# ArisKonidaris/OMLDM

Hardware: AMD Instinct MI355X
Metric: training examples/sec (whole node) + p50 predict latency, linear SVM 1/2/4/8 GPU (higher is better)
Workload: dtype fp32

## Files before the change

csrc/kernels/linear_scan3.hip:

```cpp
#include "common.h"
#include "hash_dev.h"
#include "seq_common.h"

#include <mutex>
#include <unordered_map>

namespace omldm {

typedef float f32x4 __attribute__((ext_vector_type(4)));

namespace s3 {
constexpr int CH = 64;
#ifndef OMLDM_S3_NH
#define OMLDM_S3_NH 11
#endif
constexpr int NH = OMLDM_S3_NH;
constexpr int NT = 64 * (NH + 1);
constexpr int WPE = (NH + 1 + 3) / 4;
constexpr int NHA = NH;
constexpr int GS = CH + 4;
constexpr int MAXF = 32;
constexpr int NF = (MAXF + NHA - 1) / NHA;
constexpr int KNMAX = 32;
constexpr int NJ = (KNMAX + NHA - 1) / NHA;
constexpr int MAT = CH * CH;
constexpr int RMAX = 8192;
constexpr int WS = 8;
constexpr int DS = KNMAX;
constexpr uint32_t F_TG = 1u;
constexpr uint32_t F_INIT = 2u;
constexpr uint32_t F_SCAT = 4u;
constexpr uint32_t F_SIGN = 8u;
constexpr uint32_t F_PRES = 16u;
constexpr uint32_t F_TAB = F_TG | F_INIT | F_SCAT;
constexpr int LID_SHIFT = 10;
}

template <int KN>
__host__ __device__ constexpr int s3_prep_floats() {
  return 2 * s3::MAT + s3::CH + KN * s3::CH + 3 * s3::CH;
}
template <int KN>
__host__ __device__ constexpr int s3_prep_y() {
  return 2 * s3::MAT + s3::CH + KN * s3::CH;
}
template <int KN>
__host__ __device__ constexpr int s3_prep_sg() {
  return s3_prep_y<KN>() + s3::CH;
}
template <int KN>
__host__ __device__ constexpr int s3_prep_hh() {
  return s3_prep_y<KN>() + 2 * s3::CH;
}
__device__ __forceinline__ float s3_shrink(int shr, float r, float tbase, int i, float y) {
  if (shr == 0 || y != y) return 1.f;
  if (shr == 2) {
    const float T = tbase + (float)i;
    return (T - 1.f) / T;
  }
  return r;
}

__device__ __forceinline__ void spoke_rows(int s, int R, int B, int& t0, int& t1) {
  const long long a = (long long)s * R;
  t0 = a > B ? B : (int)a;
  t1 = (a + R) > B ? B : (int)(a + R);
}

__global__ __launch_bounds__(256) void s3_slots_kernel(const void* __restrict__ src, int B,
                                                       int dc, int dn, uint32_t span, int hashed,
                                                       int cbase, int* __restrict__ slotsT) {
  __shared__ int tile[256][s3::MAXF + 1];
  const int r0 = blockIdx.x * 256, tid = threadIdx.x;
  const int nr = min(256, B - r0);
  for (int i = tid; i < nr * dc; i += 256) {
    const int r = i / dc, f = i - r * dc;
    int slot;
    if (hashed == 2) {
      const uint32_t v = reinterpret_cast<const uint16_t*>(src)[(size_t)r0 * dc + i];
      slot = v == 0xFFFFu ? -1
                          : (int)(((uint32_t)cbase + (uint32_t)f * span + (v & 0x7FFFu)) |
                                  ((v & 0x8000u) << 16));
    } else {
      const uint32_t v = reinterpret_cast<const uint32_t*>(src)[(size_t)r0 * dc + i];
      slot = hashed ? (int)v : hash_token_dev(v, f, dn, span);
    }
    tile[r][f] = slot;
  }
  __syncthreads();
  if (tid < nr)
    for (int f = 0; f < dc; ++f) slotsT[(size_t)f * B + r0 + tid] = tile[tid][f];
}

namespace s3 {
constexpr int FT = 1024;
constexpr int HCAP = 12288;
constexpr int RPT = RMAX / FT;
}

__global__ __launch_bounds__(s3::FT) void s3_flags_kernel(const int* __restrict__ slotsT, int B,
                                                          int R, uint32_t* __restrict__ meta,
                                                          int* __restrict__ lidcount, int enc,
                                                          int* __restrict__ l2s, long long gs) {
  __shared__ int hkey[s3::HCAP];
  __shared__ uint32_t hfirst[s3::HCAP];
  __shared__ uint32_t hlast[s3::HCAP];
  __shared__ int s_cnt, s_base;
  const int f = blockIdx.x, s = blockIdx.y, tid = threadIdx.x, lane = tid & 63;
  int t0, t1;
  spoke_rows(s, R, B, t0, t1);
  const int n = t1 - t0;
  if (n <= 0) return;
  for (int i = tid; i < s3::HCAP; i += s3::FT) {
    hkey[i] = -1;
    hfirst[i] = 0xFFFFFFFFu;
    hlast[i] = 0u;
  }
  if (tid == 0) s_cnt = 0;
  __syncthreads();
  const int* col = slotsT + (size_t)f * B + t0;
// ... 57 lines not shown
      const int ch = i >> 6;
      m = v[q] < 0 ? s3::F_SIGN : 0u;
      if ((last >> 6) - (first >> 6) >= 2) {
        if (ch > (first >> 6)) m |= s3::F_TG;
        if (i == first) m |= s3::F_INIT;
        if ((last >> 6) >= ch + 2) m |= s3::F_SCAT;
        m |= (uint32_t)(base + hkey[h[q]]) << s3::LID_SHIFT;
        if (l2s && lloc[q] >= 0) l2s[(size_t)s * gs + base + lloc[q]] = v[q] & 0x7fffffff;
      } else if (enc) {
        m |= s3::F_PRES | ((uint32_t)(v[q] & 0x7fffffff) << s3::LID_SHIFT);
      }
    }
    meta[(size_t)f * B + t0 + i] = m;
  }
}

__device__ __forceinline__ void s3_gram_colscale(float (*scol)[s3::CH], float cscale,
                                                 const void* __restrict__ yv, int y8, int t0,
                                                 int t1, int c, int tid) {
  if (cscale == 0.f || tid >= 2 * s3::CH) return;
  const int d = tid / s3::CH, r = tid - d * s3::CH;
  const int row = t0 + (c - d) * s3::CH + r;
  const float y = (c - d >= 0 && row < t1) ? load_y(yv, row, y8) : 0.f;
  scol[d][r] = y == y ? cscale * y : 0.f;
}

template <int KN>
__global__ __launch_bounds__(256) void s3_gram_kernel(const int* __restrict__ slotsT, int dc,
                                                      const float* __restrict__ num, int dn,
                                                      const void* __restrict__ yv, int y8,
                                                      int B, int R, int bias, int affine,
                                                      float kadd, float* __restrict__ prep,
                                                      int nchs, int shr, float shr_r,
                                                      float cscale) {
  const int c = blockIdx.x, s = blockIdx.y;
  int t0, t1;
  spoke_rows(s, R, B, t0, t1);
  if (t0 + c * s3::CH >= t1) return;
  constexpr int PF = s3_prep_floats<KN>();
  float* out = prep + ((size_t)s * nchs + c) * PF;
  __shared__ alignas(16) int sl[2][s3::MAXF][s3::CH + 4];
  __shared__ float xn[2][s3::CH][KN + 1];
  __shared__ float sa[s3::CH];
  __shared__ float scol[2][s3::CH];
  const int tid = threadIdx.x;
  s3_gram_colscale(scol, cscale, yv, y8, t0, t1, c, tid);
  for (int i = tid; i < 2 * dc * s3::CH; i += 256) {
    const int d = i / (dc * s3::CH), rem = i - d * dc * s3::CH;
    const int f = rem / s3::CH, r = rem - f * s3::CH;
    const int cc = c - d, row = t0 + cc * s3::CH + r;
    sl[d][f][r] = (cc >= 0 && row < t1) ? slotsT[(size_t)f * B + row] : -1;
  }
  for (int i = tid; i < 2 * s3::CH * KN; i += 256) {
    const int d = i / (s3::CH * KN), rem = i - d * s3::CH * KN;
    const int r = rem / KN, j = rem - r * KN;
    const int cc = c - d, row = t0 + cc * s3::CH + r;
    float x = 0.f;
    if (cc >= 0 && row < t1) x = j < dn ? num[(size_t)row * dn + j] : ((bias && j == dn) ? 1.f : 0.f);
    xn[d][r][j] = x;
  }
  __syncthreads();
  if (tid < s3::CH) {
    float n2 = 0.f;
    for (int j = 0; j < KN; ++j) n2 = fmaf(xn[0][tid][j], xn[0][tid][j], n2);
    for (int f = 0; f < dc; ++f) n2 += sl[0][f][tid] != -1 ? 1.f : 0.f;
    const bool live = t0 + c * s3::CH + tid < t1;
    const float yt = live ? load_y(yv, t0 + c * s3::CH + tid, y8) : __builtin_nanf("");
    float a = 0.f, g = 1.f;
    if (live) {
      a = affine == 1 ? (n2 > 0.f ? -1.f / (n2 + kadd) : 0.f)
        : affine == 2 ? (yt == yt ? yt : 0.f)
        : affine == 3 ? (n2 > 0.f ? 1.f / (2.f * n2 + kadd) : 0.f) : 1.f;
      if (affine == 1 && shr == 1 && yt == yt) g = 1.f / shr_r;
    }
    sa[tid] = affine == 3 ? (live ? 1.f : 0.f) : a * g;
    out[2 * s3::MAT + tid] = a;
    out[s3_prep_y<KN>() + tid] = yt;
  }
  for (int i = tid; i < KN * s3::CH; i += 256) {
    const int j = i / s3::CH, r = i - j * s3::CH;
    out[2 * s3::MAT + s3::CH + i] = xn[0][r][j];
  }
  __syncthreads();
  const int bi = tid >> 4, bj = tid & 15;
#pragma unroll 1
  for (int d = 0; d < 2; ++d) {
    float acc[4][4] = {};
    if (c - d >= 0 && !(d == 0 && bj > bi)) {
      int cnt[4][4] = {};
      for (int f = 0; f < dc; ++f) {
        const int4 a4 = *reinterpret_cast<const int4*>(&sl[0][f][4 * bi]);
        const int4 b4 = *reinterpret_cast<const int4*>(&sl[d][f][4 * bj]);
        const int av[4] = {a4.x, a4.y, a4.z, a4.w}, bv[4] = {b4.x, b4.y, b4.z, b4.w};
#pragma unroll
        for (int i = 0; i < 4; ++i) {
          const int a = av[i] == -1 ? 0x7ffffffe : av[i];
#pragma unroll
          for (int j = 0; j < 4; ++j) {
            const int x = a ^ bv[j];
            cnt[i][j] += (x & 0x7fffffff) ? 0 : (x < 0 ? -1 : 1);
          }
        }
      }
#pragma unroll
      for (int i = 0; i < 4; ++i)
#pragma unroll
        for (int j = 0; j < 4; ++j) acc[i][j] = (float)cnt[i][j];
      for (int q = 0; q < KN; ++q) {
        float xa[4], xb[4];
#pragma unroll
        for (int i = 0; i < 4; ++i) {
          xa[i] = xn[0][4 * bi + i][q];
          xb[i] = xn[d][4 * bj + i][q];
        }
#pragma unroll
        for (int i = 0; i < 4; ++i)
#pragma unroll
          for (int j = 0; j < 4; ++j) acc[i][j] = fmaf(xa[i], xb[j], acc[i][j]);
      }
    }
#pragma unroll
    for (int i = 0; i < 4; ++i) {
      const int t = 4 * bi + i;
      const float a = sa[t];
      float4 v = make_float4(a * acc[i][0], a * acc[i][1], a * acc[i][2], a * acc[i][3]);
      if (cscale != 0.f) {
        v.x *= scol[d][4 * bj + 0];
        v.y *= scol[d][4 * bj + 1];
        v.z *= scol[d][4 * bj + 2];
        v.w *= scol[d][4 * bj + 3];
      }
      if (d == 0) {
        if (4 * bj + 0 >= t) v.x = 0.f;
        if (4 * bj + 1 >= t) v.y = 0.f;
        if (4 * bj + 2 >= t) v.z = 0.f;
        if (4 * bj + 3 >= t) v.w = 0.f;
      }
      *reinterpret_cast<float4*>(&out[d * s3::MAT + t * s3::CH + 4 * bj]) = v;
    }
  }
}

__device__ int g_s3_gram_ablate = 0;

template <int KN>
__global__ __launch_bounds__(256) void s3_gram_mfma_kernel(const int* __restrict__ slotsT, int dc,
                                                           const float* __restrict__ num, int dn,
                                                           const void* __restrict__ yv, int y8,
                                                           int B, int R, int bias, int affine,
                                                           float kadd, float* __restrict__ prep,
                                                           int nchs, int shr, float shr_r,
                                                           float cscale) {
  typedef float f32x16 __attribute__((ext_vector_type(16)));
  const int c = blockIdx.x, s = blockIdx.y;
  int t0, t1;
  spoke_rows(s, R, B, t0, t1);
  if (t0 + c * s3::CH >= t1) return;
  constexpr int PF = s3_prep_floats<KN>();
  float* out = prep + ((size_t)s * nchs + c) * PF;
  __shared__ alignas(16) int sl[2][s3::MAXF][s3::CH + 4];
  __shared__ float xn[2][s3::CH][KN + 1];
  __shared__ float sa[s3::CH];
  __shared__ float scol[2][s3::CH];
  const int tid = threadIdx.x, lane = tid & 63, wave = tid >> 6;
  s3_gram_colscale(scol, cscale, yv, y8, t0, t1, c, tid);
  constexpr int NSL = 2 * s3::MAXF * s3::CH / 256, NXN = 2 * s3::CH * KN / 256;
  int sv[NSL];
  float xv[NXN];
#pragma unroll
  for (int u = 0; u < NSL; ++u) {
    const int i = tid + 256 * u;
    const int d = i / (s3::MAXF * s3::CH), rem = i - d * s3::MAXF * s3::CH;
    const int f = rem / s3::CH, r = rem - f * s3::CH;
    const int cc = c - d, row = t0 + cc * s3::CH + r;
    const bool ok = f < dc && cc >= 0 && row < t1;
    const int v = slotsT[ok ? (size_t)f * B + row : 0];
    sv[u] = ok ? v : -1;
  }
#pragma unroll
  for (int u = 0; u < NXN; ++u) {
    const int i = tid + 256 * u;
    const int d = i / (s3::CH * KN), rem = i - d * s3::CH * KN;
    const int r = rem / KN, j = rem - r * KN;
    const int cc = c - d, row = t0 + cc * s3::CH + r;
    const bool in = cc >= 0 && row < t1;
    const float x = dn > 0 ? num[(in && j < dn) ? (size_t)row * dn + j : 0] : 0.f;
    xv[u] = in ? (j < dn ? x : ((bias && j == dn) ? 1.f : 0.f)) : 0.f;
  }
#pragma unroll
  for (int u = 0; u < NSL; ++u) {
    const int i = tid + 256 * u;
    const int d = i / (s3::MAXF * s3::CH), rem = i - d * s3::MAXF * s3::CH;
    sl[d][rem / s3::CH][rem % s3::CH] = sv[u];
  }
#pragma unroll
  for (int u = 0; u < NXN; ++u) {
    const int i = tid + 256 * u;
    const int d = i / (s3::CH * KN), rem = i - d * s3::CH * KN;
    xn[d][rem / KN][rem % KN] = xv[u];
  }
  __syncthreads();
  if (tid < s3::CH) {
    float n2 = 0.f;
    for (int j = 0; j < KN; ++j) n2 = fmaf(xn[0][tid][j], xn[0][tid][j], n2);
    for (int f = 0; f < dc; ++f) n2 += sl[0][f][tid] != -1 ? 1.f : 0.f;
    const bool live = t0 + c * s3::CH + tid < t1;
    const float yt = live ? load_y(yv, t0 + c * s3::CH + tid, y8) : __builtin_nanf("");
    float a = 0.f, g = 1.f;
    if (live) {
      a = affine == 1 ? (n2 > 0.f ? -1.f / (n2 + kadd) : 0.f)
        : affine == 2 ? (yt == yt ? yt : 0.f)
        : affine == 3 ? (n2 > 0.f ? 1.f / (2.f * n2 + kadd) : 0.f) : 1.f;
      if (affine == 1 && shr == 1 && yt == yt) g = 1.f / shr_r;
    }
    sa[tid] = affine == 3 ? (live ? 1.f : 0.f) : a * g;
    out[2 * s3::MAT + tid] = a;
    out[s3_prep_y<KN>() + tid] = yt;
  }
  for (int i = tid; i < KN * s3::CH; i += 256) {
    const int j = i / s3::CH, r = i - j * s3::CH;
    out[2 * s3::MAT + s3::CH + i] = xn[0][r][j];
  }
  __syncthreads();
  const int l31 = lane & 31, hi = lane >> 5;
#pragma unroll 1
  for (int pass = 0; pass < 2; ++pass) {
    const int d = pass == 0 ? 1 : 0;
    const int I0 = pass == 0 ? 32 * (wave >> 1) : ((wave == 1 || wave == 2) ? 32 : 0);
    const int J0 = pass == 0 ? 32 * (wave & 1) : (wave >= 2 ? 32 : 0);
    const bool zero = (pass == 1 && wave == 3) || c - d < 0;
    f32x16 acc;
#pragma unroll
    for (int g = 0; g < 16; ++g) acc[g] = 0.f;
    const int abl = g_s3_gram_ablate;
    if (!zero) {
      int cnt[16];
#pragma unroll
      for (int g = 0; g < 16; ++g) cnt[g] = 0;
      for (int f = 0; f < ((abl & 1) ? 0 : dc); ++f) {
        const int b = sl[d][f][J0 + l31];
#pragma unroll
        for (int g = 0; g < 4; ++g) {
          const int4 a4 = *reinterpret_cast<const int4*>(&sl[0][f][I0 + 8 * g + 4 * hi]);
          const int av[4] = {a4.x, a4.y, a4.z, a4.w};
#pragma unroll
          for (int e = 0; e < 4; ++e) {
            const int a = av[e] == -1 ? 0x7ffffffe : av[e];
            const int x = a ^ b;
            cnt[4 * g + e] += (x & 0x7fffffff) ? 0 : (x < 0 ? -1 : 1);
          }
        }
      }
#pragma unroll
      for (int g = 0; g < 16; ++g) acc[g] = (float)cnt[g];
      if (!(abl & 2)) {
#pragma unroll
        for (int k0 = 0; k0 < KN; k0 += 2)
          acc = __builtin_amdgcn_mfma_f32_32x32x2f32(xn[0][I0 + l31][k0 + hi],
                                                     xn[d][J0 + l31][k0 + hi], acc, 0, 0, 0);
      }
    }
    if (abl & 4) continue;
#pragma unroll
    for (int g = 0; g < 16; ++g) {
      const int t = I0 + (g & 3) + 8 * (g >> 2) + 4 * hi, col = J0 + l31;
      float v = sa[t] * acc[g];
      if (cscale != 0.f) v *= scol[d][col];
      if (d == 0 && col >= t) v = 0.f;
      out[d * s3::MAT + t * s3::CH + col] = v;
    }
  }
}

template <int KN>
__global__ __launch_bounds__(64) void s3_sigma_kernel(float* __restrict__ prep, int nchs, int B,
                                                      int R, int shr, float shr_r, float tbase,
                                                      float* __restrict__ sig) {
  constexpr int PF = s3_prep_floats<KN>();
  const int s = blockIdx.x, lane = threadIdx.x;
  int t0, t1;
  spoke_rows(s, R, B, t0, t1);
  const int n = t1 - t0;
  if (n <= 0) return;
  float* P0 = prep + (size_t)s * nchs * PF;
  auto at = [&](int i) -> float* { return P0 + (size_t)(i >> 6) * PF + (i & 63); };
  const int L = (n + 63) / 64, i0 = lane * L, i1 = min(n, i0 + L);
  float pr = 1.f;
  for (int i = i0; i < i1; ++i) pr *= s3_shrink(shr, shr_r, tbase, i, at(i)[s3_prep_y<KN>()]);
  float incl = pr;
#pragma unroll
  for (int d = 1; d < 64; d <<= 1) {
    const float o = __shfl_up(incl, d, 64);
    if (lane >= d) incl *= o;
  }
  float sg = __shfl_up(incl, 1, 64);
  if (lane == 0) sg = 1.f;
  for (int i = i0; i < i1; ++i) {
    float* b = at(i);
    b[s3_prep_sg<KN>()] = sg;
    sg *= s3_shrink(shr, shr_r, tbase, i, b[s3_prep_y<KN>()]);
    b[s3_prep_hh<KN>()] = 1.f / sg;
  }
  const int tail = (64 - (n & 63)) & 63;
  if (lane < tail) {
    float* b = at(n + lane);
    b[s3_prep_sg<KN>()] = 1.f;
    b[s3_prep_hh<KN>()] = 1.f;
  }
  if (lane == 63) sig[s] = incl;
}

struct S3Smem {
  alignas(16) float G[2][s3::CH][s3::GS];
  alignas(16) float X1[2][s3::CH][s3::GS];
  float part[2][s3::NHA][s3::CH];
  float cb[2][s3::CH];
  int last;
};

template <int RULE>
struct S3Cand {
  float lo, hi, d;
  __device__ __forceinline__ float operator()(float u, const SeqParams& p, float y) const {
    if constexpr (RULE == kSeqHinge) {
      return __builtin_amdgcn_fmed3f(u, lo, hi);
    } else if constexpr (RULE == kSeqEps) {
      return __builtin_amdgcn_fmed3f(u, 0.f, hi) + __builtin_amdgcn_fmed3f(u + d, lo, 0.f);
    } else if constexpr (RULE == kSeqPegasos) {
      return u < lo ? hi : 0.f;
    } else {
      return hi * __builtin_amdgcn_rcpf(1.f + __expf(lo * u));
    }
  }
};

__device__ unsigned long long* g_s3_stamps;
__device__ int g_s3_debug;
__device__ unsigned long long* g_s3mc_dbg;
__device__ int g_s3_comb_err;
__device__ int g_s3_dense_order = 0;
__device__ int g_s3_hprio = 0;

typedef __attribute__((address_space(1))) unsigned long long s3_gu64;
template <bool B>
struct S3Tag {
  static constexpr bool value = B;
};
struct S3Comb {
  const int* lidcount;
  unsigned long long* gran;
  uint32_t epoch;
  int S_act;
// ... 286 lines not shown
        const int sl = i < n ? slot[u] : 0;
        d[u] -= i < n ? (cb.wbf ? s3_w16(w, sl) : w[sl]) : 0.f;
      }
    }
#pragma unroll
    for (int u = 0; u < FB; ++u) {
      const int i = i0 + u * s3::NT;
      if (i < n && d[u] != 0.f) atomicAdd(&cb.dacc[slot[u]], sc * d[u]);
    }
  }
}

__device__ __forceinline__ void s3_spoke_end(bool tail, const int* __restrict__ slotsT, int dc,
                                             int B, int R, const S3Comb& cb,
                                             const float* __restrict__ ws,
                                             const float* __restrict__ wsd, int dn, int dim,
                                             const SeqParams& p, S3Smem& sm, int s) {
  if (tail) {
    __syncthreads();
    s3_combine_spoke(slotsT, dc, B, R, cb, sm, s, 0, 1);
  }
  s3_scan_arrive(cb, ws, wsd, dn, dim, p, sm);
}

template <int RULE, int KN, bool RARE>
__device__ __forceinline__ void s3_scan_body(
    int bid, int nblk, int tail, S3Smem& sm, float* tab,
    const int* __restrict__ slotsT, const uint32_t* __restrict__ meta, int dc, int dn,
    const void* __restrict__ yv, int B, int R, const float* __restrict__ prep, int nchs,
    const float* __restrict__ w, int dim, float* __restrict__ aglob, int cap, long long gstride,
    const S3Comb& cb, float* __restrict__ ws, float* __restrict__ wsd, const SeqParams& p,
    unsigned long long* __restrict__ rgran) {
  constexpr int PF = s3_prep_floats<KN>();
  if (bid >= cb.S_act) {
    if (RARE && bid < 2 * cb.S_act) {
      s3_rare(slotsT, dc, B, R, w, cb, rgran, sm, bid - cb.S_act);
      if (cb.inscan == 2) s3_fold_pres(meta, dc, B, R, cb, bid - cb.S_act);
      if (tail == 2) {
        __syncthreads();
        s3_combine_spoke(slotsT, dc, B, R, cb, sm, bid - cb.S_act, 0, 1);
      }
      return;
    }
    s3_combine(slotsT, dc, B, R, cb, sm, (RARE ? 2 : 1) * cb.S_act, bid, nblk, cb.cns);
    return;
  }
  const int tid = threadIdx.x;
  const int wave = __builtin_amdgcn_readfirstlane(tid >> 6), lane = tid & 63;
  const int s = bid;
  int t0, t1;
  spoke_rows(s, R, B, t0, t1);
  if (t0 >= t1) {
    if (tid < s3::WS) ws[(size_t)s * s3::WS + tid] = 0.f;
    if (tid < s3::DS) wsd[(size_t)s * s3::DS + tid] = 0.f;
    s3_scan_arrive(cb, ws, wsd, dn, dim, p, sm);
    return;
  }
  const int nch = (t1 - t0 + s3::CH - 1) / s3::CH;
  const float* P0 = prep + (size_t)s * nchs * PF;
  auto chunk_prep = [&](int k) { return P0 + (size_t)k * PF; };
  float* ag = aglob + (size_t)s * gstride;

  unsigned long long* stamps = g_s3_stamps;
  const bool dbg_gather = g_s3_debug == 1;
  unsigned long long st_acc[12] = {};
  unsigned long long st_t = stamps ? clock64() : 0;
  auto stamp = [&](int k) {
    if (stamps) {
      const unsigned long long now = clock64();
      st_acc[k] += now - st_t;
      st_t = now;
    }
  };

  if (wave == 0) {
    __builtin_amdgcn_s_setprio(3);
    float loss = 0.f, nex = 0.f, mist = 0.f, sqe = 0.f;
    float f1 = 0.f;
    float ynx = chunk_prep(0)[s3_prep_y<KN>() + lane];
    float anx = chunk_prep(0)[2 * s3::MAT + lane];
    const bool shr = p.shr != 0;
    float snx = shr ? chunk_prep(0)[s3_prep_sg<KN>() + lane] : 1.f;
    float hnx = shr ? chunk_prep(0)[s3_prep_hh<KN>() + lane] : 1.f;
    for (int k = -1; k <= nch; ++k) {
      if (k >= 0 && k < nch) {
        const int b = k & 1;
        const int row = t0 + k * s3::CH + lane;
        const bool valid = row < t1 && ynx == ynx;
        const float y = valid ? ynx : 0.f;
        const float a = valid ? anx : 0.f;
        const float sg = valid ? snx : 1.f, hh = valid ? hnx : 1.f;
        if (k + 1 < nch) {
          ynx = chunk_prep(k + 1)[s3_prep_y<KN>() + lane];
          anx = chunk_prep(k + 1)[2 * s3::MAT + lane];
          if (shr) {
            snx = chunk_prep(k + 1)[s3_prep_sg<KN>() + lane];
            hnx = chunk_prep(k + 1)[s3_prep_hh<KN>() + lane];
          }
        }
        float m0 = 0.f;
#pragma unroll
        for (int q = 0; q < s3::NHA; ++q) m0 += sm.part[b][q][lane];
        S3Cand<RULE> cf;
        float u, bc = 0.f;
        const float inv = -a;
        if constexpr (RULE == kSeqHinge) {
          bc = y * inv * hh;
          cf.lo = y < 0.f ? -p.cclip * hh : 0.f;
          cf.hi = y < 0.f ? 0.f : (y > 0.f ? p.cclip * hh : 0.f);
          u = fmaf(a * (sg * hh), m0, bc) + f1;
        } else if constexpr (RULE == kSeqEps) {
          bc = (y - p.eps) * inv * hh;
          cf.d = 2.f * p.eps * inv * hh;
          cf.lo = valid ? -p.cclip * hh : 0.f;
          cf.hi = valid ? p.cclip * hh : 0.f;
          u = fmaf(a * (sg * hh), m0, bc) + f1;
        } else if constexpr (RULE == kSeqPegasos) {
          const float T = p.tbase + (float)(row - t0);
          cf.lo = valid ? 1.f / sg : 0.f;
          cf.hi = valid ? y * hh / (p.lam * T) : 0.f;
          u = fmaf(a, m0, 0.f) + f1;
        } else {
          cf.lo = y * sg;
          cf.hi = p.lr * y * hh;
          u = m0 + f1;
        }
        const float* grow = &sm.G[b][lane][0];
        const float* xrow = &sm.X1[b ^ 1][lane][0];
        float gg[s3::CH], xx[s3::CH];
#pragma unroll
        for (int t4 = 0; t4 < s3::CH; t4 += 4) {
          const float4 g4 = *reinterpret_cast<const float4*>(grow + t4);
          const float4 x4 = *reinterpret_cast<const float4*>(xrow + t4);
          gg[t4] = g4.x, gg[t4 + 1] = g4.y, gg[t4 + 2] = g4.z, gg[t4 + 3] = g4.w;
          xx[t4] = x4.x, xx[t4 + 1] = x4.y, xx[t4 + 2] = x4.z, xx[t4 + 3] = x4.w;
        }
        stamp(8);
        float n1 = 0.f;
        auto chain = [&](auto step) {
#pragma unroll
          for (int t = 0; t < s3::CH; ++t) {
            const float ct = readlane_f(step(u), t);
            u = fmaf(ct, gg[t], u);
            n1 = fmaf(ct, xx[t], n1);
            asm volatile("" : "+v"(u), "+v"(n1));
          }
        };
        if constexpr (RULE == kSeqLogistic) {
          if (!shr) {
            const float lo2 = y * 1.44269504088896341f;
            chain([&](float v) {
              return __builtin_amdgcn_rcpf(1.f + __builtin_amdgcn_exp2f(lo2 * v));
            });
          } else {
            chain([&](float v) { return cf(v, p, y); });
          }
        } else {
          chain([&](float v) { return cf(v, p, y); });
        }
        stamp(9);
        const float c = cf(u, p, y);
        sm.cb[b][lane] = c;
        if (row < t1 && cb.inscan != 1)
          __hip_atomic_store((s3_gu64*)(cb.gran + row),
                             ((unsigned long long)cb.epoch << 32) | __float_as_uint(c),
                             __ATOMIC_RELAXED, __HIP_MEMORY_SCOPE_AGENT);
        if (valid) {
          float m;
          if constexpr (RULE == kSeqLogistic) m = sg * u;
          else if constexpr (RULE == kSeqPegasos) m = sg * y * u;
          else m = inv > 0.f ? (bc - u) * __builtin_amdgcn_rcpf(inv * hh) : 0.f;
          seq_stats<RULE>(m, y, p, loss, mist, sqe);
          nex += 1.f;
        }
        f1 = n1;
      }
      stamp(0);
      __syncthreads();
      stamp(1);
    }
    if (stamps && lane == 0)
      for (int q = 0; q < 12; ++q)
        if (q < 2 || q >= 8) atomicAdd(&stamps[(size_t)s * 16 + q], st_acc[q]);
    loss = wave_sum(loss);
    nex = wave_sum(nex);
    mist = wave_sum(mist);
    sqe = wave_sum(sqe);
    if (lane == 0) {
      float* wr = ws + (size_t)s * s3::WS;
      wr[0] = loss;
      wr[1] = nex;
      wr[2] = mist;
      wr[3] = sqe;
      wr[4] = 1.f;
      wr[5] = 0.f;
      wr[6] = 0.f;
      wr[7] = 0.f;
    }
    if (cb.inscan) s3_inscan_flush<RARE>(cb, tab, ag, cap, w, s);
    s3_spoke_end(tail == 1, slotsT, dc, B, R, cb, ws, wsd, dn, dim, p, sm, s);
    return;
  }

  const int q = wave - 1, r = lane;
  const int swave = g_s3_debug >= 16 ? g_s3_debug - 16 : 1;
  if (g_s3_hprio) {
    if (q >= 7) __builtin_amdgcn_s_setprio(2);
    else if (q >= 3) __builtin_amdgcn_s_setprio(1);
  }
  const int qd = g_s3_dense_order ? s3::NHA - 1 - q : q;
  const int kd = dn + (p.bias ? 1 : 0);
  const int hl = q * 64 + lane;
  const bool inscan = cb.inscan != 0, inscan1 = cb.inscan == 1;
  const uint32_t tmask = inscan ? s3::F_TAB : s3::F_SCAT;
  const float isc = inscan1 ? cb.inv_p * (cb.sig ? cb.sig[s] : 1.f) : 0.f;
  float wn[s3::NJ], w0[s3::NJ];
#pragma unroll
  for (int i = 0; i < s3::NJ; ++i) {
    const int j = qd + s3::NHA * i;
    const int jw = j < dn ? j : dim - 1;
    const float wj = cb.wbf ? s3_w16(w, jw) : w[jw];
    w0[i] = (j < KN && (j < dn || (p.bias && j == dn))) ? wj : 0.f;
    wn[i] = w0[i];
  }
  constexpr int NV4 = (2 * s3::MAT / 4 + 64 * s3::NHA - 1) / (64 * s3::NHA);
  struct Set {
    int cs[s3::NF];
    uint32_t cm[s3::NF];
    float g[s3::NF];
    f32x4 v[NV4];
    float xs[s3::NJ], xc[s3::NJ];
    unsigned long long rg;
  };
  uint32_t p1[s3::NF], p2[s3::NF];
  const unsigned long long want = (unsigned long long)cb.epoch;
  bool dead = false;
  auto load_rare = [&](int ch) -> unsigned long long {
    const int row = t0 + ch * s3::CH + r;
    const bool ok = RARE && q == 0 && ch >= 0 && ch < nch && row < t1;
    return ok ? __hip_atomic_load((s3_gu64*)(rgran + row), __ATOMIC_RELAXED,
                                  __HIP_MEMORY_SCOPE_AGENT)
              : (want << 32);
  };
  auto load_words = [&](int ch, Set& S) {
    if constexpr (RARE) {
      S.rg = load_rare(ch);
#pragma unroll
      for (int i = 0; i < s3::NF; ++i) {
        const int f = q + s3::NHA * i;
        const int row = t0 + ch * s3::CH + r;
        const bool ok = ch >= 0 && ch < nch && f < dc && row < t1;
        const uint32_t mm = meta[ok ? (size_t)f * B + row : 0];
        S.cm[i] = ok ? mm : 0u;
        S.cs[i] = ok && (mm & (s3::F_TG | s3::F_INIT)) ? 0 : -1;
      }
      return;
    }
#pragma unroll
    for (int i = 0; i < s3::NF; ++i) {
      const int f = q + s3::NHA * i;
      const int row = t0 + ch * s3::CH + r;
      const bool ok = ch >= 0 && ch < nch && f < dc && row < t1;
      const size_t at = ok ? (size_t)f * B + row : 0;
      const int sl = slotsT[at];
      const uint32_t mm = meta[at];
      S.cs[i] = ok ? sl : -1;
      S.cm[i] = ok ? mm : 0u;
    }
  };
  auto issue_gathers = [&](Set& S) {
    if constexpr (RARE) return;
    if (cb.wbf) {
#pragma unroll
      for (int i = 0; i < s3::NF; ++i) {
        const bool glob = !RARE && S.cs[i] != -1 && !(S.cm[i] & s3::F_TG);
        S.g[i] = s3_w16(w, (glob && !dbg_gather) ? (S.cs[i] & 0x7fffffff) : 0);
      }
      return;
    }
#pragma unroll
    for (int i = 0; i < s3::NF; ++i) {
      const bool glob = !RARE && S.cs[i] != -1 && !(S.cm[i] & s3::F_TG);
      S.g[i] = w[(glob && !dbg_gather) ? (S.cs[i] & 0x7fffffff) : 0];
    }
  };
  auto issue_staging = [&](int ch, Set& S) {
#pragma unroll
    for (int u = 0; u < NV4; ++u) {
      const int i = min(hl + 64 * s3::NHA * u, 2 * s3::MAT / 4 - 1);
      const int mtx = i >> 10, e = i & 1023;
      const int kc = max(0, min(ch + mtx, nch - 1));
      S.v[u] = reinterpret_cast<const f32x4*>(chunk_prep(kc) + mtx * s3::MAT)[e];
    }
  };
  constexpr int NJK = (KN + s3::NHA - 1) / s3::NHA;
  auto load_dense = [&](int ch, float* xd) {
#pragma unroll
    for (int i = 0; i < NJK; ++i) {
      const int j = qd + s3::NHA * i;
      const bool ok = j < KN && ch >= 0 && ch < nch;
      const int jc = j < KN ? j : 0, cc = max(0, min(ch, nch - 1));
      const float v = chunk_prep(cc)[2 * s3::MAT + s3::CH + jc * s3::CH + r];
      xd[i] = ok ? v : 0.f;
    }
  };
  auto body = [&](auto spill_tag, int k, Set& CUR, Set& NXT) {
    constexpr bool SPILL = decltype(spill_tag)::value;
    const int cn = k + 1, ks = k - 1;
    if (wave == swave) stamp(7);
    load_words(cn + 1, NXT);
    issue_staging(cn + 1, NXT);
    load_dense(ks + 1, NXT.xs);
    load_dense(cn + 1, NXT.xc);
    if (wave == swave) stamp(3);
    if (ks >= 0) {
      const float cv = sm.cb[ks & 1][r];
#pragma unroll
      for (int i = 0; i < s3::NF; ++i) {
        const uint32_t m = p2[i];
        const bool sc = (m & tmask) != 0u && cv != 0.f;
        const bool dr = inscan1 && (m & s3::F_PRES) != 0u && cv != 0.f;
        if (__builtin_amdgcn_ballot_w64(sc || dr) == 0ull) continue;
        const int lid = (int)(m >> s3::LID_SHIFT);
        const float val = (m & s3::F_SIGN) ? -cv : cv;
        if (dr) atomicAdd(&cb.dacc[lid], val * isc);
        if (sc) {
          if constexpr (SPILL) {
            if (lid < cap) atomicAdd(&tab[lid], val);
            else atomicAdd(&ag[lid - cap], val);
          } else {
            atomicAdd(&tab[lid], val);
          }
        }
      }
#pragma unroll
      for (int i = 0; i < NJK; ++i) {
        const int j = qd + s3::NHA * i;
        if (j < kd) wn[i] += wave_sum(cv * CUR.xs[i]);
      }
    }
    if (wave == swave) stamp(6);
    if (cn < nch) {
      float base = 0.f;
#pragma unroll
      for (int i = 0; i < NJK; ++i) base = fmaf(CUR.xc[i], wn[i], base);
      if constexpr (RARE) {
        if (q == 0) {
          for (unsigned spins = 0;
               __builtin_amdgcn_ballot_w64((CUR.rg >> 32) != want) != 0ull;) {
            if (dead || ++spins > s3::SPIN_MAX) {
              if (!dead && r == 0) atomicExch(&g_s3_comb_err, 2);
              dead = true;
              break;
            }
            __builtin_amdgcn_s_sleep(1);
            CUR.rg = load_rare(cn);
          }
          base += (CUR.rg >> 32) == want ? __uint_as_float((uint32_t)CUR.rg) : 0.f;
        }
      }
      if constexpr (!SPILL) {
        float tv[s3::NF];
#pragma unroll
        for (int i = 0; i < s3::NF; ++i) {
          const uint32_t m = CUR.cm[i];
          const bool tg = CUR.cs[i] != -1 && (m & s3::F_TG);
          tv[i] = 0.f;
          if (tg) tv[i] = tab[(int)(m >> s3::LID_SHIFT)];
        }
#pragma unroll
        for (int i = 0; i < s3::NF; ++i) {
          const uint32_t m = CUR.cm[i];
          const bool here = CUR.cs[i] != -1;
          const bool tg = here && (m & s3::F_TG), init = here && !tg && (m & s3::F_INIT);
          const float val = tg ? tv[i] : (RARE ? 0.f : CUR.g[i]);
          if (init) tab[(int)(m >> s3::LID_SHIFT)] = val;
          if (here && (!RARE || tg)) base += (m & s3::F_SIGN) ? -val : val;
        }
      }
#pragma unroll
      for (int i = 0; SPILL && i < s3::NF; ++i) {
        const uint32_t m = CUR.cm[i];
        const bool here = CUR.cs[i] != -1;
        const int lid = (int)(m >> s3::LID_SHIFT);
        const bool tg = here && (m & s3::F_TG), init = here && !tg && (m & s3::F_INIT);
        float val = RARE ? 0.f : CUR.g[i];
        if (!SPILL || __builtin_amdgcn_ballot_w64((tg || init) && lid >= cap) == 0ull) {
          if (tg) val = tab[lid];
          if (init) tab[lid] = val;
        } else if constexpr (SPILL) {
          if (tg) val = lid < cap ? tab[lid] : __hip_atomic_load(&ag[lid - cap], __ATOMIC_RELAXED,
                                                                 __HIP_MEMORY_SCOPE_WORKGROUP);
          if (init) {
            if (lid < cap) tab[lid] = val;
            else __hip_atomic_store(&ag[lid - cap], val, __ATOMIC_RELAXED,
                                    __HIP_MEMORY_SCOPE_WORKGROUP);
          }
          asm volatile("s_waitcnt vmcnt(0)" ::: "memory");
        }
        if (here && (!RARE || tg)) base += (m & s3::F_SIGN) ? -val : val;
      }
      sm.part[cn & 1][q][r] = base;
    }
    if (wave == swave) stamp(4);
#pragma unroll
    for (int u = 0; u < NV4; ++u) {
      const int i = hl + 64 * s3::NHA * u;
      const int mtx = i >> 10, e = i & 1023;
      if (i < 2 * s3::MAT / 4 && cn + mtx < nch) {
        const int row = e >> 4, col = (e & 15) * 4;
        float* dst = mtx == 0 ? &sm.G[cn & 1][row][col] : &sm.X1[(cn + 1) & 1][row][col];
        *reinterpret_cast<f32x4*>(dst) = CUR.v[u];
      }
    }
    issue_gathers(NXT);
#pragma unroll
    for (int i = 0; i < s3::NF; ++i) {
      p2[i] = p1[i];
      p1[i] = CUR.cm[i];
    }
    if (wave == swave) stamp(5);
    __syncthreads();
  };

  Set A, Bs;
#pragma unroll
  for (int i = 0; i < s3::NF; ++i) p1[i] = p2[i] = 0u;
  load_words(0, A);
  issue_staging(0, A);
  load_dense(-2, A.xs);
  load_dense(0, A.xc);
  issue_gathers(A);
  if (cb.lidcount[s] <= cap) {
    for (int k = -1; k <= nch; k += 2) {
      body(S3Tag<false>{}, k, A, Bs);
      if (k + 1 <= nch) body(S3Tag<false>{}, k + 1, Bs, A);
    }
  } else {
    for (int k = -1; k <= nch; k += 2) {
      body(S3Tag<true>{}, k, A, Bs);
      if (k + 1 <= nch) body(S3Tag<true>{}, k + 1, Bs, A);
    }
  }
  if (stamps && lane == 0 && wave == swave)
    for (int k = 2; k < 8; ++k) atomicAdd(&stamps[(size_t)s * 16 + k], st_acc[k]);
#pragma unroll
  for (int i = 0; i < s3::NJ; ++i) {
    const int j = qd + s3::NHA * i;
    if (lane == 0 && j < KN) wsd[(size_t)s * s3::DS + j] = wn[i] - w0[i];
  }
  if (q == 0 && lane >= KN && lane < s3::DS) wsd[(size_t)s * s3::DS + lane] = 0.f;
  if (cb.inscan) s3_inscan_flush<RARE>(cb, tab, ag, cap, w, s);
  s3_spoke_end(tail == 1, slotsT, dc, B, R, cb, ws, wsd, dn, dim, p, sm, s);
}

constexpr int kS3MaxPipes = 16;
struct S3Pipe {
  const float* w;
  float* aglob;
  float* ws;
  float* wsd;
  unsigned long long* rgran;
  S3Comb cb;
  SeqParams p;
};
struct S3Pipes {
  int M;
  int ncomb;
  int tail;
  const unsigned long long* wflag;
  unsigned long long wepoch;
  S3Pipe pipe[kS3MaxPipes];
};

__global__ void s3_signal_kernel(unsigned long long* flag, unsigned long long epoch) {
  if (threadIdx.x == 0)
    __hip_atomic_store(flag, epoch, __ATOMIC_RELEASE, __HIP_MEMORY_SCOPE_AGENT);
}

__device__ __forceinline__ void s3_wait_prep(const unsigned long long* flag,
                                             unsigned long long epoch) {
  if (flag == nullptr) return;
  if (threadIdx.x == 0) {
    for (unsigned spins = 0;
         __hip_atomic_load(flag, __ATOMIC_RELAXED, __HIP_MEMORY_SCOPE_AGENT) < epoch;) {
      if (++spins > s3::SPIN_MAX) {
        atomicExch(&g_s3_comb_err, 3);
        break;
      }
      __builtin_amdgcn_s_sleep(2);
    }
    __builtin_amdgcn_fence(__ATOMIC_ACQUIRE, "agent");
  }
  __syncthreads();
}

template <int RULE, int KN, bool RARE>
__global__ __launch_bounds__(s3::NT, s3::WPE) __attribute__((amdgpu_waves_per_eu(s3::WPE, s3::WPE))) void s3_scan_kernel(
    const int* __restrict__ slotsT, const uint32_t* __restrict__ meta, int dc, int dn,
    const void* __restrict__ yv, int B, int R, const float* __restrict__ prep, int nchs,
    int dim, int cap, long long gstride, int S_act, S3Pipes pp) {
  __shared__ S3Smem sm;
  extern __shared__ float tab[];
  const int nblk = s3_nper(S_act, RARE, pp.ncomb, pp.pipe[0].cb.cns);
  const int pi = (int)blockIdx.x / nblk, local = (int)blockIdx.x % nblk;
  s3_wait_prep(pp.wflag, pp.wepoch);
  int bid;
  if (RARE && local < S_act) bid = S_act + local;
  else if (RARE && local < 2 * S_act) bid = local - S_act;
  else bid = local;
  const S3Pipe& P = pp.pipe[pi];
  s3_scan_body<RULE, KN, RARE>(bid, nblk, pp.tail, sm, tab, slotsT, meta,
// ... 330 lines not shown
  auto w0_at = [&](int i, int c) {
    const int j = q + s3::NHA * i;
    const int key = j < dn ? j : dim - 1;
    const bool real = j < KN && (j < dn || (bias && j == dn));
    return real ? A.Wt[(size_t)key * A.kp + c] : 0.f;
  };
#pragma unroll
  for (int i = 0; i < NJK0; ++i)
#pragma unroll
    for (int c = 0; c < K; ++c) wn[c][i] = w0_at(i, c);
  constexpr int NV4 = (2 * s3::MAT / 4 + 64 * s3::NHA - 1) / (64 * s3::NHA);
  constexpr int NJK = (KN + s3::NHA - 1) / s3::NHA;
  struct Set {
    int cs[s3::NF];
    uint32_t cm[s3::NF];
    float g[s3::NF][K];
    f32x4 v[NV4];
    float xs[s3::NJ], xc[s3::NJ];
  };
  uint32_t p1[s3::NF], p2[s3::NF];
  auto load_words = [&](int ch, Set& S) {
#pragma unroll
    for (int i = 0; i < s3::NF; ++i) {
      const int f = q + s3::NHA * i;
      const int row = t0 + ch * s3::CH + r;
      const bool ok = ch >= 0 && ch < nch && f < dc && row < t1;
      const size_t at = ok ? (size_t)f * B + row : 0;
      const int sl = slotsT[at];
      const uint32_t mm = meta[at];
      S.cs[i] = ok ? sl : -1;
      S.cm[i] = ok ? mm : 0u;
    }
  };
  auto issue_gathers = [&](Set& S) {
#pragma unroll
    for (int i = 0; i < s3::NF; ++i) {
      const bool glob = S.cs[i] != -1 && !(S.cm[i] & s3::F_TG);
      const float* src = A.Wt + (size_t)(glob ? (S.cs[i] & 0x7fffffff) : 0) * A.kp;
      if constexpr (K >= 4) {
#pragma unroll
        for (int c4 = 0; c4 < K; c4 += 4) {
          const float4 v = *reinterpret_cast<const float4*>(src + c4);
          S.g[i][c4] = v.x, S.g[i][c4 + 1] = v.y, S.g[i][c4 + 2] = v.z, S.g[i][c4 + 3] = v.w;
        }
      } else {
        const float2 v = *reinterpret_cast<const float2*>(src);
        S.g[i][0] = v.x, S.g[i][1] = v.y;
      }
    }
  };
  auto issue_staging = [&](int ch, Set& S) {
#pragma unroll
    for (int u = 0; u < NV4; ++u) {
      const int i = min(hl + 64 * s3::NHA * u, 2 * s3::MAT / 4 - 1);
      const int mtx = i >> 10, e = i & 1023;
      const int kc = max(0, min(ch + mtx, nch - 1));
      S.v[u] = reinterpret_cast<const f32x4*>(chunk_prep(kc) + mtx * s3::MAT)[e];
    }
  };
  auto load_dense = [&](int ch, float* xd) {
#pragma unroll
    for (int i = 0; i < NJK; ++i) {
      const int j = q + s3::NHA * i;
      const bool ok = j < KN && ch >= 0 && ch < nch;
      const int jc = j < KN ? j : 0, cc = max(0, min(ch, nch - 1));
      const float v = chunk_prep(cc)[2 * s3::MAT + s3::CH + jc * s3::CH + r];
      xd[i] = ok ? v : 0.f;
    }
  };
  auto tab_add = [&](auto spill_tag, int lid, int c, float v) {
    constexpr bool SPILL = decltype(spill_tag)::value;
    if (!SPILL || lid < capid) atomicAdd(&tab[lid * K + c], v);
    else atomicAdd(&ag[(size_t)(lid - capid) * K + c], v);
  };
  unsigned long long* const hdbg = g_s3mc_dbg;
  unsigned long long h_sc = 0, h_mg = 0, h_st = 0, h_wt = 0;
  constexpr bool LEAN = K >= 8;
  auto store_staging = [&](int cn, const Set& S) {
#pragma unroll
    for (int u = 0; u < NV4; ++u) {
      const int i = hl + 64 * s3::NHA * u;
      const int mtx = i >> 10, e = i & 1023;
      if (i < 2 * s3::MAT / 4 && cn + mtx < nch) {
        const int row = e >> 4, col = (e & 15) * 4;
        float* dst = mtx == 0 ? &sm.G[cn & 1][row][col] : &sm.X1[(cn + 1) & 1][row][col];
        *reinterpret_cast<f32x4*>(dst) = S.v[u];
      }
    }
  };
  auto body = [&](auto spill_tag, int k, Set& CUR, Set& NXT) {
    constexpr bool SPILL = decltype(spill_tag)::value;
    const int cn = k + 1, ks = k - 1;
    const unsigned long long ha = hdbg ? __builtin_amdgcn_s_memtime() : 0;
    load_words(cn + 1, NXT);
    if constexpr (LEAN) {
      issue_staging(cn, CUR);
      if constexpr (K < 16) issue_gathers(CUR);
    } else {
      issue_staging(cn + 1, NXT);
    }
    load_dense(ks + 1, NXT.xs);
    load_dense(cn + 1, NXT.xc);
    if (ks >= 0) {
      const float tv = sm.tau[ks & 1][r];
      const int rc = sm.rr[ks & 1][r];
      const float yf = chunk_prep(ks)[s3_prep_y<KN>() + r];
      const int yc = (yf == yf && yf >= 0.f && yf < (float)A.nclass) ? (int)yf : -1;
#pragma unroll
      for (int i = 0; i < s3::NF; ++i) {
        const uint32_t m = p2[i];
        const bool sc = (m & s3::F_SCAT) != 0u && tv != 0.f;
        if (__builtin_amdgcn_ballot_w64(sc) == 0ull) continue;
        const int lid = (int)(m >> s3::LID_SHIFT);
        const float val = (m & s3::F_SIGN) ? -tv : tv;
        if (sc) {
          if (yc >= 0) tab_add(spill_tag, lid, yc, val);
          if (rc >= 0) tab_add(spill_tag, lid, rc, -val);
        }
      }
      if constexpr (SPILL) asm volatile("s_waitcnt vmcnt(0)" ::: "memory");
#pragma unroll
      for (int i = 0; i < NJK; ++i) {
        const int j = q + s3::NHA * i;
        if (j < kd) {
#pragma unroll
          for (int c = 0; c < K; ++c) {
            if (K <= 4 || c < A.nclass) {
              const float cf = c == yc ? tv : (c == rc ? -tv : 0.f);
              wn[c][i] += wave_sum(cf * CUR.xs[i]);
            }
          }
        }
      }
    }
    if constexpr (LEAN) store_staging(cn, CUR);
    const unsigned long long hb = hdbg ? __builtin_amdgcn_s_memtime() : 0;
    if (cn < nch) {
      float base[K];
#pragma unroll
      for (int c = 0; c < K; ++c) {
        base[c] = 0.f;
#pragma unroll
        for (int i = 0; i < NJK; ++i) base[c] = fmaf(CUR.xc[i], wn[c][i], base[c]);
      }
#pragma unroll
      for (int i = 0; i < s3::NF; ++i) {
        const uint32_t m = CUR.cm[i];
        const bool here = CUR.cs[i] != -1;
        const bool tg = here && (m & s3::F_TG), init = here && !tg && (m & s3::F_INIT);
        const int lid = (int)(m >> s3::LID_SHIFT);
        float val[K];
        if constexpr (K >= 16) {
          const bool glob = here && !(m & s3::F_TG);
          const float* src = A.Wt + (size_t)(glob ? (CUR.cs[i] & 0x7fffffff) : 0) * A.kp;
#pragma unroll
          for (int c4 = 0; c4 < K; c4 += 4) {
            const float4 v = *reinterpret_cast<const float4*>(src + c4);
            val[c4] = v.x, val[c4 + 1] = v.y, val[c4 + 2] = v.z, val[c4 + 3] = v.w;
          }
        } else {
#pragma unroll
          for (int c = 0; c < K; ++c) val[c] = CUR.g[i][c];
        }
        if (!SPILL || __builtin_amdgcn_ballot_w64((tg || init) && lid >= capid) == 0ull) {
          if (tg) {
#pragma unroll
            for (int c = 0; c < K; ++c) val[c] = tab[lid * K + c];
// ... 645 lines not shown
```

Before: 345.1 million.

## Stream gram matrices from global memory directly into scan-wave registers

Changes the prep gram/X1 matrix layout to a column-quad-major order (s3_mat_at) so each lane can read its row as contiguous f32x4 vectors. The scan wave now loads the G and X1 rows for the next chunk straight from global memory into registers, interleaved with the sequential chain, instead of having all waves stage the matrices through LDS each chunk. This drops the staging loads/stores and their LDS traffic from the gather waves, but puts global-load latency on the serial scan wave's critical path and adds register pressure. The multi-chunk staging path's index mapping is adjusted for the new layout.

```diff
diff --git a/csrc/kernels/linear_scan3.hip b/csrc/kernels/linear_scan3.hip
--- a/csrc/kernels/linear_scan3.hip
+++ b/csrc/kernels/linear_scan3.hip
@@ -36,6 +36,10 @@
 constexpr int LID_SHIFT = 10;
 }
 
+__host__ __device__ constexpr int s3_mat_at(int t, int col) {
+  return ((col >> 2) * s3::CH + t) * 4 + (col & 3);
+}
+
 template <int KN>
 __host__ __device__ constexpr int s3_prep_floats() {
   return 2 * s3::MAT + s3::CH + KN * s3::CH + 3 * s3::CH;
@@ -259,7 +263,7 @@
     out[2 * s3::MAT + s3::CH + i] = xn[0][r][j];
   }
   __syncthreads();
-  const int bi = tid >> 4, bj = tid & 15;
+  const int bi = tid & 15, bj = tid >> 4;
 #pragma unroll 1
   for (int d = 0; d < 2; ++d) {
     float acc[4][4] = {};
@@ -313,7 +317,7 @@
         if (4 * bj + 2 >= t) v.z = 0.f;
         if (4 * bj + 3 >= t) v.w = 0.f;
       }
-      *reinterpret_cast<float4*>(&out[d * s3::MAT + t * s3::CH + 4 * bj]) = v;
+      *reinterpret_cast<float4*>(&out[d * s3::MAT + s3_mat_at(t, 4 * bj)]) = v;
     }
   }
 }
@@ -415,10 +419,10 @@
 #pragma unroll
       for (int g = 0; g < 16; ++g) cnt[g] = 0;
       for (int f = 0; f < ((abl & 1) ? 0 : dc); ++f) {
-        const int b = sl[d][f][J0 + l31];
+        const int b = sl[0][f][I0 + l31];
 #pragma unroll
         for (int g = 0; g < 4; ++g) {
-          const int4 a4 = *reinterpret_cast<const int4*>(&sl[0][f][I0 + 8 * g + 4 * hi]);
+          const int4 a4 = *reinterpret_cast<const int4*>(&sl[d][f][J0 + 8 * g + 4 * hi]);
           const int av[4] = {a4.x, a4.y, a4.z, a4.w};
 #pragma unroll
           for (int e = 0; e < 4; ++e) {
@@ -433,18 +437,25 @@
       if (!(abl & 2)) {
 #pragma unroll
         for (int k0 = 0; k0 < KN; k0 += 2)
-          acc = __builtin_amdgcn_mfma_f32_32x32x2f32(xn[0][I0 + l31][k0 + hi],
-                                                     xn[d][J0 + l31][k0 + hi], acc, 0, 0, 0);
+          acc = __builtin_amdgcn_mfma_f32_32x32x2f32(xn[d][J0 + l31][k0 + hi],
+                                                     xn[0][I0 + l31][k0 + hi], acc, 0, 0, 0);
       }
     }
     if (abl & 4) continue;
-#pragma unroll
-    for (int g = 0; g < 16; ++g) {
-      const int t = I0 + (g & 3) + 8 * (g >> 2) + 4 * hi, col = J0 + l31;
-      float v = sa[t] * acc[g];
-      if (cscale != 0.f) v *= scol[d][col];
-      if (d == 0 && col >= t) v = 0.f;
-      out[d * s3::MAT + t * s3::CH + col] = v;
+    const int t = I0 + l31;
+    const float at = sa[t];
+#pragma unroll
+    for (int g4 = 0; g4 < 4; ++g4) {
+      const int col0 = J0 + 8 * g4 + 4 * hi;
+      float v[4];
+#pragma unroll
+      for (int e = 0; e < 4; ++e) {
+        v[e] = at * acc[4 * g4 + e];
+        if (cscale != 0.f) v[e] *= scol[d][col0 + e];
+        if (d == 0 && col0 + e >= t) v[e] = 0.f;
+      }
+      *reinterpret_cast<float4*>(&out[d * s3::MAT + s3_mat_at(t, col0)]) =
+          make_float4(v[0], v[1], v[2], v[3]);
     }
   }
 }
@@ -897,22 +908,53 @@
     const bool shr = p.shr != 0;
     float snx = shr ? chunk_prep(0)[s3_prep_sg<KN>() + lane] : 1.f;
     float hnx = shr ? chunk_prep(0)[s3_prep_hh<KN>() + lane] : 1.f;
-    for (int k = -1; k <= nch; ++k) {
-      if (k >= 0 && k < nch) {
+    auto mat_rows = [&](int kc, int mtx) {
+      return reinterpret_cast<const f32x4*>(chunk_prep(min(kc, nch - 1)) + mtx * s3::MAT);
+    };
+    const unsigned ul = (unsigned)lane;
+    auto sbase = [](const float* p) {
+      asm volatile("" : "+s"(p));
+      return (const __attribute__((address_space(1))) float*)p;
+    };
+    auto sbase4 = [](const f32x4* p) {
+      asm volatile("" : "+s"(p));
+      return (const __attribute__((address_space(1))) f32x4*)p;
+    };
+    auto scan_chunks = [&](auto plain_tag) {
+    constexpr bool PLAIN = decltype(plain_tag)::value;
+    f32x4 g4[s3::CH / 4], x4[s3::CH / 4];
+    {
+      const f32x4* pg = mat_rows(0, 0);
+      const f32x4* px = mat_rows(1, 1);
+#pragma unroll
+      for (int c = 0; c < s3::CH / 4; ++c) {
+        x4[c] = sbase4(px + c * s3::CH)[ul];
+        g4[c] = sbase4(pg + c * s3::CH)[ul];
+      }
+    }
+    stamp(0);
+    __syncthreads();
+    stamp(1);
+    for (int k = 0; k < nch; ++k) {
+      {
         const int b = k & 1;
         const int row = t0 + k * s3::CH + lane;
         const bool valid = row < t1 && ynx == ynx;
         const float y = valid ? ynx : 0.f;
         const float a = valid ? anx : 0.f;
         const float sg = valid ? snx : 1.f, hh = valid ? hnx : 1.f;
-        if (k + 1 < nch) {
-          ynx = chunk_prep(k + 1)[s3_prep_y<KN>() + lane];
-          anx = chunk_prep(k + 1)[2 * s3::MAT + lane];
+        {
+          const float* pn = chunk_prep(min(k + 1, nch - 1));
+          const auto* py = sbase(pn + s3_prep_y<KN>());
+          ynx = py[ul];
+          anx = sbase(pn + 2 * s3::MAT)[ul];
           if (shr) {
-            snx = chunk_prep(k + 1)[s3_prep_sg<KN>() + lane];
-            hnx = chunk_prep(k + 1)[s3_prep_hh<KN>() + lane];
+            snx = py[s3::CH + ul];
+            hnx = py[2 * s3::CH + ul];
           }
         }
+        const f32x4* pg = mat_rows(k + 1, 0);
+        const f32x4* px = mat_rows(k + 2, 1);
         float m0 = 0.f;
 #pragma unroll
         for (int q = 0; q < s3::NHA; ++q) m0 += sm.part[b][q][lane];
@@ -940,36 +982,32 @@
           cf.hi = p.lr * y * hh;
           u = m0 + f1;
         }
-        const float* grow = &sm.G[b][lane][0];
-        const float* xrow = &sm.X1[b ^ 1][lane][0];
-        float gg[s3::CH], xx[s3::CH];
-#pragma unroll
-        for (int t4 = 0; t4 < s3::CH; t4 += 4) {
-          const float4 g4 = *reinterpret_cast<const float4*>(grow + t4);
-          const float4 x4 = *reinterpret_cast<const float4*>(xrow + t4);
-          gg[t4] = g4.x, gg[t4 + 1] = g4.y, gg[t4 + 2] = g4.z, gg[t4 + 3] = g4.w;
-          xx[t4] = x4.x, xx[t4 + 1] = x4.y, xx[t4 + 2] = x4.z, xx[t4 + 3] = x4.w;
-        }
         stamp(8);
         float n1 = 0.f;
         auto chain = [&](auto step) {
+          const __attribute__((address_space(1))) f32x4 *pgb = nullptr, *pxb = nullptr;
 #pragma unroll
           for (int t = 0; t < s3::CH; ++t) {
             const float ct = readlane_f(step(u), t);
-            u = fmaf(ct, gg[t], u);
-            n1 = fmaf(ct, xx[t], n1);
+            u = fmaf(ct, g4[t >> 2][t & 3], u);
+            n1 = fmaf(ct, x4[t >> 2][t & 3], n1);
             asm volatile("" : "+v"(u), "+v"(n1));
+            if ((t & 3) == 3) {
+              const int c = t >> 2;
+              if ((c & 3) == 0) {
+                pxb = sbase4(px + c * s3::CH);
+                pgb = sbase4(pg + c * s3::CH);
+              }
+              x4[c] = pxb[(c & 3) * s3::CH + ul];
+              g4[c] = pgb[(c & 3) * s3::CH + ul];
+            }
           }
         };
-        if constexpr (RULE == kSeqLogistic) {
-          if (!shr) {
-            const float lo2 = y * 1.44269504088896341f;
-            chain([&](float v) {
-              return __builtin_amdgcn_rcpf(1.f + __builtin_amdgcn_exp2f(lo2 * v));
-            });
-          } else {
-            chain([&](float v) { return cf(v, p, y); });
-          }
+        if constexpr (PLAIN) {
+          const float lo2 = y * 1.44269504088896341f;
+          chain([&](float v) {
+            return __builtin_amdgcn_rcpf(1.f + __builtin_amdgcn_exp2f(lo2 * v));
+          });
         } else {
           chain([&](float v) { return cf(v, p, y); });
         }
@@ -994,6 +1032,15 @@
       __syncthreads();
       stamp(1);
     }
+    };
+    if (RULE == kSeqLogistic && !shr) {
+      if constexpr (RULE == kSeqLogistic) scan_chunks(S3Tag<true>{});
+    } else {
+      scan_chunks(S3Tag<false>{});
+    }
+    stamp(0);
+    __syncthreads();
+    stamp(1);
     if (stamps && lane == 0)
       for (int q = 0; q < 12; ++q)
         if (q < 2 || q >= 8) atomicAdd(&stamps[(size_t)s * 16 + q], st_acc[q]);
@@ -1025,7 +1072,6 @@
   }
   const int qd = g_s3_dense_order ? s3::NHA - 1 - q : q;
   const int kd = dn + (p.bias ? 1 : 0);
-  const int hl = q * 64 + lane;
   const bool inscan = cb.inscan != 0, inscan1 = cb.inscan == 1;
   const uint32_t tmask = inscan ? s3::F_TAB : s3::F_SCAT;
   const float isc = inscan1 ? cb.inv_p * (cb.sig ? cb.sig[s] : 1.f) : 0.f;
@@ -1038,12 +1084,10 @@
     w0[i] = (j < KN && (j < dn || (p.bias && j == dn))) ? wj : 0.f;
     wn[i] = w0[i];
   }
-  constexpr int NV4 = (2 * s3::MAT / 4 + 64 * s3::NHA - 1) / (64 * s3::NHA);
   struct Set {
     int cs[s3::NF];
     uint32_t cm[s3::NF];
     float g[s3::NF];
-    f32x4 v[NV4];
     float xs[s3::NJ], xc[s3::NJ];
     unsigned long long rg;
   };
@@ -1099,15 +1143,6 @@
       S.g[i] = w[(glob && !dbg_gather) ? (S.cs[i] & 0x7fffffff) : 0];
     }
   };
-  auto issue_staging = [&](int ch, Set& S) {
-#pragma unroll
-    for (int u = 0; u < NV4; ++u) {
-      const int i = min(hl + 64 * s3::NHA * u, 2 * s3::MAT / 4 - 1);
-      const int mtx = i >> 10, e = i & 1023;
-      const int kc = max(0, min(ch + mtx, nch - 1));
-      S.v[u] = reinterpret_cast<const f32x4*>(chunk_prep(kc) + mtx * s3::MAT)[e];
-    }
-  };
   constexpr int NJK = (KN + s3::NHA - 1) / s3::NHA;
   auto load_dense = [&](int ch, float* xd) {
 #pragma unroll
@@ -1124,7 +1159,6 @@
     const int cn = k + 1, ks = k - 1;
     if (wave == swave) stamp(7);
     load_words(cn + 1, NXT);
-    issue_staging(cn + 1, NXT);
     load_dense(ks + 1, NXT.xs);
     load_dense(cn + 1, NXT.xc);
     if (wave == swave) stamp(3);
@@ -1218,23 +1252,12 @@
       sm.part[cn & 1][q][r] = base;
     }
     if (wave == swave) stamp(4);
-#pragma unroll
-    for (int u = 0; u < NV4; ++u) {
-      const int i = hl + 64 * s3::NHA * u;
-      const int mtx = i >> 10, e = i & 1023;
-      if (i < 2 * s3::MAT / 4 && cn + mtx < nch) {
-        const int row = e >> 4, col = (e & 15) * 4;
-        float* dst = mtx == 0 ? &sm.G[cn & 1][row][col] : &sm.X1[(cn + 1) & 1][row][col];
-        *reinterpret_cast<f32x4*>(dst) = CUR.v[u];
-      }
-    }
     issue_gathers(NXT);
 #pragma unroll
     for (int i = 0; i < s3::NF; ++i) {
       p2[i] = p1[i];
       p1[i] = CUR.cm[i];
     }
-    if (wave == swave) stamp(5);
     __syncthreads();
   };
 
@@ -1242,7 +1265,6 @@
 #pragma unroll
   for (int i = 0; i < s3::NF; ++i) p1[i] = p2[i] = 0u;
   load_words(0, A);
-  issue_staging(0, A);
   load_dense(-2, A.xs);
   load_dense(0, A.xc);
   issue_gathers(A);
@@ -1739,7 +1761,7 @@
       const int i = hl + 64 * s3::NHA * u;
       const int mtx = i >> 10, e = i & 1023;
       if (i < 2 * s3::MAT / 4 && cn + mtx < nch) {
-        const int row = e >> 4, col = (e & 15) * 4;
+        const int row = e & 63, col = (e >> 6) * 4;
         float* dst = mtx == 0 ? &sm.G[cn & 1][row][col] : &sm.X1[(cn + 1) & 1][row][col];
         *reinterpret_cast<f32x4*>(dst) = S.v[u];
       }
```

Result: no change. 345.6 million (median of 2 runs) (+0.2%).
